# nmwsharp/diffusion-net

Measured on AMD Instinct MI355X. Metric: vertices/sec fwd+bwd, C_width=128 K=128, higher is better.
Workload: dtype f32; 1 GPU; train step (fwd+NLL+bwd+Adam) on a ragged batch of 16 meshes x ~10000 vertices per GPU, DiffusionNet C_in=3 C_out=8 C_width=128 K=128 N_block=4 outputs_at=faces dropout=on; meshes_per_gpu=16, verts_per_gpu_step=158481, parallelism=dp1, streams_per_gpu=1, step_mode=HIP-graph replay

## Files before the change

### diffusion-net_amd/csrc/dn_tn_da.hip

```cpp
#include "dn_common.h"
#include <string.h>

#define DN_DA_THREADS 512
#define DN_DA_KS 16
#define DN_DA_ROWB 576
#define DN_DA_PLANE (DN_DA_KS * DN_DA_ROWB)
#define DN_DA_BUF (6 * DN_DA_PLANE)
#define DN_DA_LDS (128 * 1024)

struct DaRegs {
    float4 dd, gx, gy;
    float live;
};

__device__ __forceinline__ void da_load(const DaArgs& g, long long r_beg, long long r_end, int step, int kr, int q, DaRegs& R) {
    const long long row = r_beg + (long long)step * DN_DA_KS + kr;
    const bool ok = row < r_end;
    const long long off = (ok ? row : r_beg) * 128 + 4 * q;
    R.live = ok ? 1.f : 0.f;
    R.dd = *reinterpret_cast<const float4*>(g.dd + off);
    R.gx = *reinterpret_cast<const float4*>(g.gx + off);
    R.gy = *reinterpret_cast<const float4*>(g.gy + off);
}

template <int NP>
__device__ __forceinline__ void da_put(unsigned char* planes, int off, float4 v, float s) {
    uint2 pl[NP];
    dn_split_f4<NP>(v, s, pl);
#pragma unroll
    for (int p = 0; p < NP; ++p) *reinterpret_cast<uint2*>(planes + p * DN_DA_PLANE + off) = pl[p];
}

template <int NP>
__device__ __forceinline__ void da_store(unsigned char* buf, int kr, int q, const DaRegs& R, float sa, float sb) {
    const float4 bx = dn_f4_scale(R.gx, R.live), by = dn_f4_scale(R.gy, R.live);
    const float4 ax = dn_f4_mul(R.dd, bx), ay = dn_f4_mul(R.dd, by);
    const int off = kr * DN_DA_ROWB + q * 8;
    da_put<NP>(buf, off, ax, sa);
    da_put<NP>(buf, off + 256, ay, sa);
    da_put<NP>(buf + 3 * DN_DA_PLANE, off, bx, sb);
    da_put<NP>(buf + 3 * DN_DA_PLANE, off + 256, by, sb);
}

__device__ __forceinline__ uint4 da_frag(const unsigned char* p) {
    const uint2 lo = dn_lds_tr16(p), hi = dn_lds_tr16(p + 4 * DN_DA_ROWB);
    return make_uint4(lo.x, lo.y, hi.x, hi.y);
}

template <int NP>
__device__ __forceinline__ void da_compute(const unsigned char* buf, int wr, int wc, int lane, f32x16 (&acc)[4][2]) {
    const int g = lane >> 4, c = lane & 15;
    const int lane_off = (8 * (g >> 1) + (c >> 2)) * DN_DA_ROWB + (16 * (g & 1) + 4 * (c & 3)) * 2;
    const unsigned char* sA = buf + lane_off + wr * 256;
    const unsigned char* sB = buf + 3 * DN_DA_PLANE + lane_off + wc * 128;
    uint4 b[NP][2];
#pragma unroll
    for (int p = 0; p < NP; ++p)
#pragma unroll
        for (int nt = 0; nt < 2; ++nt) b[p][nt] = da_frag(sB + p * DN_DA_PLANE + nt * 64);
#pragma unroll
    for (int mt = 0; mt < 4; ++mt) {
        uint4 a[NP];
#pragma unroll
        for (int p = 0; p < NP; ++p) a[p] = da_frag(sA + p * DN_DA_PLANE + mt * 64);
        constexpr int NPROD = NP == 3 ? 6 : 3;
        constexpr int PA[6] = {NP == 3 ? 1 : 0, NP == 3 ? 0 : 1, NP == 3 ? 2 : 0, 0, 1, 0};
        constexpr int PB[6] = {1, NP == 3 ? 2 : 0, 0, 1, 0, 0};
#pragma unroll
        for (int p = 0; p < NPROD; ++p)
#pragma unroll
            for (int nt = 0; nt < 2; ++nt) {
                if constexpr (NP == 3) acc[mt][nt] = dn_mfma_bf16(a[PA[p]], b[PB[p]][nt], acc[mt][nt]);
                else acc[mt][nt] = dn_mfma_f16(a[PA[p]], b[PB[p]][nt], acc[mt][nt]);
            }
    }
}

DN_CLK_DECLARE(tn_da)
template <int NP>
__global__ __launch_bounds__(DN_DA_THREADS) DN_WAVES_PER_EU(2) void tngemm_da_kernel(DaArgs g) {
    DN_CLK_STAMP(tn_da, 0);
    float sa = 1.f, sb = 1.f, so = 1.f;
    if constexpr (NP == 2) {
        sa = dn_pow2_scale(dn_amax_eval(g.a_amax));
        sb = dn_pow2_scale(dn_amax_eval(g.b_amax));
        so = (1.f / sa) * (1.f / sb);
    }
    DN_DYN_SMEM(smem_raw);
    unsigned char* smem = reinterpret_cast<unsigned char*>(smem_raw);
    const int tid = threadIdx.x, lane = tid & 63, wave = tid >> 6;
    const int wr = wave >> 2, wc = wave & 3;
    const int kr = tid >> 5, q = tid & 31;

    const long long r_beg = (long long)blockIdx.x * g.rows_per_wg;
    const long long r_end = (r_beg + g.rows_per_wg < g.V) ? r_beg + g.rows_per_wg : g.V;
    const int nsteps = r_end > r_beg ? (int)((r_end - r_beg + DN_DA_KS - 1) / DN_DA_KS) : 0;

    f32x16 acc[4][2];
#pragma unroll
    for (int i = 0; i < 4; ++i)
#pragma unroll
        for (int j = 0; j < 2; ++j)
#pragma unroll
            for (int r = 0; r < 16; ++r) acc[i][j][r] = 0.f;

    if (nsteps > 0) {
        DaRegs R0, R1;
        da_load(g, r_beg, r_end, 0, kr, q, R0);
        da_load(g, r_beg, r_end, 1, kr, q, R1);
        da_store<NP>(smem, kr, q, R0, sa, sb);
        da_load(g, r_beg, r_end, 2, kr, q, R0);
        __syncthreads();
        for (int s = 0; s < nsteps; s += 2) {
            da_store<NP>(smem + DN_DA_BUF, kr, q, R1, sa, sb);
            da_load(g, r_beg, r_end, s + 3, kr, q, R1);
            da_compute<NP>(smem, wr, wc, lane, acc);
            __syncthreads();
            if (s + 1 < nsteps) {
                da_store<NP>(smem, kr, q, R0, sa, sb);
                da_load(g, r_beg, r_end, s + 4, kr, q, R0);
                da_compute<NP>(smem + DN_DA_BUF, wr, wc, lane, acc);
                __syncthreads();
            }
        }
    }
    __syncthreads();

    float* ex = reinterpret_cast<float*>(smem);
    if (wc >= 2) {
        float* mine = ex + (size_t)(wr * 2 + (wc - 2)) * 8 * 16 * 64;
#pragma unroll
        for (int mt = 0; mt < 4; ++mt)
#pragma unroll
            for (int nt = 0; nt < 2; ++nt)
#pragma unroll
                for (int r = 0; r < 16; ++r) mine[((mt * 2 + nt) * 16 + r) * 64 + lane] = acc[mt][nt][r];
    }
    __syncthreads();
    if (wc < 2) {
        const float* theirs = ex + (size_t)((1 - wr) * 2 + wc) * 8 * 16 * 64;
        const float sgn = wr == 0 ? 1.f : -1.f;
        float* out = g.partial + ((long long)blockIdx.x * 2 + wr) * 128 * 128;
        const int li = lane & 31;
#pragma unroll
        for (int mt = 0; mt < 4; ++mt)
#pragma unroll
            for (int nt = 0; nt < 2; ++nt)
#pragma unroll
                for (int r = 0; r < 16; ++r) {
                    const int o = mt * 32 + dn_acc_row(r, lane), c = wc * 64 + nt * 32 + li;
                    const float v = acc[mt][nt][r] + sgn * theirs[((mt * 2 + nt) * 16 + r) * 64 + lane];
                    out[o * 128 + c] = NP == 2 ? v * so : v;
                }
    }
    DN_CLK_STAMP(tn_da, 1);
}

int dn_launch_tn_da(const float* dd, const float* gx, const float* gy, long long V, float* partial, int nwg, hipStream_t stream,
                    const float* dd_amax, const float* g_amax) {
    if (V <= 0 || nwg <= 0) return DN_ERR_BAD_MODE;
    DaArgs g;
    memset(&g, 0, sizeof(g));
    g.dd = dd; g.gx = gx; g.gy = gy; g.partial = partial; g.V = V;
    g.f16 = (dd_amax && g_amax) ? 1 : 0;
    g.a_amax.p[0] = dd_amax; g.a_amax.mul = g_amax; g.b_amax.p[0] = g_amax;
    const long long per = (V + nwg - 1) / nwg;
    g.rows_per_wg = (int)((per + DN_DA_KS - 1) / DN_DA_KS * DN_DA_KS);
#ifndef DN_EMULATE
    static unsigned long long lds_opt_in = 0;
    { const int oe_ = dn_lds_opt_in(reinterpret_cast<const void*>(&tngemm_da_kernel<3>), DN_DA_LDS, &lds_opt_in); if (oe_) return oe_; }
    static unsigned long long lds_opt_in2 = 0;
    { const int oe_ = dn_lds_opt_in(reinterpret_cast<const void*>(&tngemm_da_kernel<2>), DN_DA_LDS, &lds_opt_in2); if (oe_) return oe_; }
#endif
    dn_prof_begin(DN_K_TN_DA, stream);
    if (g.f16) DN_LAUNCH(tngemm_da_kernel<2>, dim3(nwg, 1, 1), dim3(DN_DA_THREADS, 1, 1), DN_DA_LDS, stream, g);
    else DN_LAUNCH(tngemm_da_kernel<3>, dim3(nwg, 1, 1), dim3(DN_DA_THREADS, 1, 1), DN_DA_LDS, stream, g);
    dn_prof_end(DN_K_TN_DA, stream, 8.0 * (double)V * 128.0 * 128.0, 4.0 * (3.0 * (double)V * 128.0 + 2.0 * nwg * 128.0 * 128.0));
    return (int)hipGetLastError();
}
```

Baseline: 32.79 million vertices/s.

## Interleave LDS split-stores with MFMA in DA tn-gemm via scheduling group barriers

New measurement: 32.86 million vertices/s, median of 6. Within noise of the previous version (+0.2%).

```diff
diff --git a/diffusion-net_amd/csrc/dn_tn_da.hip b/diffusion-net_amd/csrc/dn_tn_da.hip
--- a/diffusion-net_amd/csrc/dn_tn_da.hip
+++ b/diffusion-net_amd/csrc/dn_tn_da.hip
@@ -76,6 +76,81 @@
     }
 }
 
+#ifdef DN_EMULATE
+#define DN_DA_SCHED(mask, n, id)
+#define DN_DA_SCHED_FENCE()
+#define DN_DA_MFMA_ORDER()
+#else
+#define DN_DA_MFMA_ORDER() __builtin_amdgcn_sched_barrier(0x7F6)
+#define DN_DA_SCHED(mask, n, id) __builtin_amdgcn_sched_group_barrier(mask, n, id)
+#define DN_DA_SCHED_FENCE() __builtin_amdgcn_sched_barrier(0)
+#endif
+#define DN_DA_SG_VALU 0x2
+#define DN_DA_SG_MFMA 0x8
+#define DN_DA_SG_DS_READ 0x100
+#define DN_DA_SG_DS_WRITE 0x200
+template <int NP, int MT>
+__device__ __forceinline__ void da_pin_group() {
+    constexpr int NMFMA = NP == 3 ? 12 : 6, SPLIT_VALU = NP == 3 ? 22 : 12;
+#pragma unroll
+    for (int i = 0; i < NMFMA; ++i) {
+        DN_DA_SCHED(DN_DA_SG_MFMA, 1, MT + 1);
+        DN_DA_SCHED(DN_DA_SG_VALU, (SPLIT_VALU + NMFMA - 1) / NMFMA, MT + 1);
+        if (MT < 3 && i < 2 * NP) DN_DA_SCHED(DN_DA_SG_DS_READ, 1, MT + 1);
+        if (i >= NMFMA - NP) DN_DA_SCHED(DN_DA_SG_DS_WRITE, 1, MT + 1);
+    }
+}
+template <int NP>
+__device__ __forceinline__ void da_step(const unsigned char* __restrict__ cur, unsigned char* __restrict__ nxt, int kr, int q, const DaRegs& R,
+                                        float sa, float sb, int wr, int wc, int lane, f32x16 (&acc)[4][2]) {
+    const int g = lane >> 4, c = lane & 15;
+    const int lane_off = (8 * (g >> 1) + (c >> 2)) * DN_DA_ROWB + (16 * (g & 1) + 4 * (c & 3)) * 2;
+    const unsigned char* sA = cur + lane_off + wr * 256;
+    const unsigned char* sB = cur + 3 * DN_DA_PLANE + lane_off + wc * 128;
+    const int off = kr * DN_DA_ROWB + q * 8;
+    constexpr int NPROD = NP == 3 ? 6 : 3;
+    constexpr int PA[6] = {NP == 3 ? 1 : 0, NP == 3 ? 0 : 1, NP == 3 ? 2 : 0, 0, 1, 0};
+    constexpr int PB[6] = {1, NP == 3 ? 2 : 0, 0, 1, 0, 0};
+
+    float4 v[4];
+    v[0] = dn_f4_scale(R.gx, R.live); v[1] = dn_f4_scale(R.gy, R.live);
+    v[2] = dn_f4_mul(R.dd, v[0]);     v[3] = dn_f4_mul(R.dd, v[1]);
+
+    uint4 b[NP][2], a[2][NP];
+#pragma unroll
+    for (int p = 0; p < NP; ++p)
+#pragma unroll
+        for (int nt = 0; nt < 2; ++nt) b[p][nt] = da_frag(sB + p * DN_DA_PLANE + nt * 64);
+#pragma unroll
+    for (int p = 0; p < NP; ++p) a[0][p] = da_frag(sA + p * DN_DA_PLANE);
+    DN_DA_SCHED(DN_DA_SG_VALU, 16, 0);
+    DN_DA_SCHED(DN_DA_SG_DS_READ, 6 * NP, 0);
+#pragma unroll
+    for (int mt = 0; mt < 4; ++mt) {
+        uint2 pl[NP];
+        dn_split_f4<NP>(v[mt], mt < 2 ? sb : sa, pl);
+        if (mt < 3) {
+#pragma unroll
+            for (int p = 0; p < NP; ++p) a[(mt + 1) & 1][p] = da_frag(sA + p * DN_DA_PLANE + (mt + 1) * 64);
+        }
+#pragma unroll
+        for (int p = 0; p < NPROD; ++p)
+#pragma unroll
+            for (int nt = 0; nt < 2; ++nt) {
+                if constexpr (NP == 3) acc[mt][nt] = dn_mfma_bf16(a[mt & 1][PA[p]], b[PB[p]][nt], acc[mt][nt]);
+                else acc[mt][nt] = dn_mfma_f16(a[mt & 1][PA[p]], b[PB[p]][nt], acc[mt][nt]);
+                DN_DA_MFMA_ORDER();
+            }
+        unsigned char* dst = nxt + (mt < 2 ? 3 * DN_DA_PLANE : 0) + off + (mt & 1) * 256;
+#pragma unroll
+        for (int p = 0; p < NP; ++p) *reinterpret_cast<uint2*>(dst + p * DN_DA_PLANE) = pl[p];
+        if (mt == 0) da_pin_group<NP, 0>();
+        else if (mt == 1) da_pin_group<NP, 1>();
+        else if (mt == 2) da_pin_group<NP, 2>();
+        else da_pin_group<NP, 3>();
+    }
+}
+
 DN_CLK_DECLARE(tn_da)
 template <int NP>
 __global__ __launch_bounds__(DN_DA_THREADS) DN_WAVES_PER_EU(2) void tngemm_da_kernel(DaArgs g) {
@@ -111,18 +186,17 @@
         da_store<NP>(smem, kr, q, R0, sa, sb);
         da_load(g, r_beg, r_end, 2, kr, q, R0);
         __syncthreads();
-        for (int s = 0; s < nsteps; s += 2) {
-            da_store<NP>(smem + DN_DA_BUF, kr, q, R1, sa, sb);
+        for (int s = 0; s + 1 < nsteps; s += 2) {
+            da_step<NP>(smem, smem + DN_DA_BUF, kr, q, R1, sa, sb, wr, wc, lane, acc);
             da_load(g, r_beg, r_end, s + 3, kr, q, R1);
-            da_compute<NP>(smem, wr, wc, lane, acc);
+            DN_DA_SCHED_FENCE();
             __syncthreads();
-            if (s + 1 < nsteps) {
-                da_store<NP>(smem, kr, q, R0, sa, sb);
-                da_load(g, r_beg, r_end, s + 4, kr, q, R0);
-                da_compute<NP>(smem + DN_DA_BUF, wr, wc, lane, acc);
-                __syncthreads();
-            }
+            da_step<NP>(smem + DN_DA_BUF, smem, kr, q, R0, sa, sb, wr, wc, lane, acc);
+            da_load(g, r_beg, r_end, s + 4, kr, q, R0);
+            DN_DA_SCHED_FENCE();
+            __syncthreads();
         }
+        if (nsteps & 1) da_compute<NP>(smem, wr, wc, lane, acc);
     }
     __syncthreads();
 
```
